# haasn/libplacebo

Measured on AMD Instinct MI355X. Metric: Mpixels/s (and frames/s) for EWA-Lánczos 1080p→4K + HDR tonemap, 1/2/4/8 GPU, higher is better.
Workload: dtype f32; 1 GPU; ewa_1080p_to_4k_hdr_tonemap; src=1920x1080 rgba16, dst=3840x2160 rgba16, pool=10, api=pl_render_image, measured=output Mpixels/s through pl_render_image, one independent stream per GPU, render_errors=0, parallelism=1 independent stream(s), one per GPU

## Files before the change

### libplacebo_amd/csrc/hip/backend.h

```cpp
#ifndef PLH_BACKEND_H_
#define PLH_BACKEND_H_

#include <stddef.h>
#include <stdint.h>

#include "plh_device.h"

#ifdef __cplusplus
extern "C" {
#endif

struct plh_dev_info {
    char name[256];
    char arch[64];
    int compute_units;
    int wavefront_size;
    size_t lds_per_block;
    size_t total_mem;
    int clock_khz;
    uint8_t uuid[16];
    int pci_domain, pci_bus, pci_device;
};

int plh_dev_count(void);
const char *plh_strerror(int err);
int plh_dev_open(int device, struct plh_dev_info *info);
int plh_stream_create(int device, plh_stream *out);
int plh_stream_device(plh_stream s, int *cus);
int plh_kernel_needs_lds(const void *kernel, plh_stream s, size_t bytes, uint64_t *done);
const void *plh_pqseg_tables(plh_stream s, const float consts[5]);
void plh_stream_destroy(plh_stream s);
int plh_stream_sync(plh_stream s);
int plh_stream_idle(plh_stream s);

void *plh_malloc(int device, size_t size);
void plh_free(void *ptr);
void *plh_host_alloc(size_t size);
void *plh_host_alloc_coherent(size_t size);
void plh_host_free(void *ptr);

int plh_copy2d_h2d(plh_stream s, void *dst, size_t dpitch, const void *src, size_t spitch,
                   size_t row_bytes, size_t rows);
int plh_copy2d_d2h(plh_stream s, void *dst, size_t dpitch, const void *src, size_t spitch,
                   size_t row_bytes, size_t rows);
int plh_copy2d_d2d(plh_stream s, void *dst, size_t dpitch, const void *src, size_t spitch,
// ... 27 lines not shown
```

### libplacebo_amd/csrc/hip/backend.hip

```cpp
#include <hip/hip_runtime.h>
#include <string.h>

#include "backend.h"
#include "devmath.hiph"

#define CHK(x) do { hipError_t e_ = (x); if (e_ != hipSuccess) return -(int) e_; } while (0)

extern "C" {

int plh_dev_count(void)
{
    int n = 0;
    if (hipGetDeviceCount(&n) != hipSuccess)
        return 0;
    return n;
}

const char *plh_strerror(int err)
{
    if (err == -1000)
        return "LDS tile does not fit";
    if (err == -1003)
        return "frame mixing ops need a plain (nearest / bilinear) sampler";
    if (err == -1005)
// ... 296 lines not shown

extern "C" int plh_launch_clear_tiles(plh_stream s, const struct plh_view *dst, const float c0[4],
                                      const float c1[4], float kx, float ky)
{
    const dim3 block(64, 4), grid((dst->w + 63) / 64, (dst->h + 3) / 4);
    const float4_t a = { c0[0], c0[1], c0[2], c0[3] }, b = { c1[0], c1[1], c1[2], c1[3] };
    hipLaunchKernelGGL(k_clear_tiles, grid, block, 0, (hipStream_t) s, *dst, a, b, kx, ky);
    const hipError_t err = hipGetLastError();
    return err == hipSuccess ? 0 : -(int) err;
}

#include <math.h>
#include <mutex>
#include "pqseg.hiph"

static double pqseg_oetf(double x, double m1, double c3, double m2)
{
    const double a = (double) PQ_A;
    const double y = x > 0.0 ? pow(x, m1) : 0.0;
    const double w = a * (1.0 - y) / (1.0 + c3 * y);
    return exp(m2 * log1p(-w));
}

static double pqseg_eotf(double v, double c3, double inv_m2, double inv_m1)
{
    const double a = (double) PQ_A;
    if (!(v > 0.0))
        return 0.0;
    const double u = -expm1(log(v) * inv_m2);
    double inner = (a - u) / (a + c3 * u);
    if (!(inner > 0.0))
        return 0.0;
    return pow(inner, inv_m1);
}

static void pqseg_fit(const double node[4], const double f[4], float out[4])
{
    double d[4] = { f[0], f[1], f[2], f[3] };
    for (int j = 1; j < 4; j++) {
        for (int i = 3; i >= j; i--)
            d[i] = (d[i] - d[i - 1]) / (node[i] - node[i - j]);
    }
    double c[4] = { d[3], 0.0, 0.0, 0.0 };
    int deg = 0;
    for (int j = 2; j >= 0; j--) {
// ... 1 lines not shown
        for (int i = 0; i <= deg; i++) {
            n[i] += c[i];
            n[i + 1] -= c[i] * node[j];
        }
        deg++;
        n[deg] += d[j];
        for (int i = 0; i <= deg; i++)
            c[i] = n[i];
    }
    out[0] = (float) c[3];
    out[1] = (float) c[2];
    out[2] = (float) c[1];
    out[3] = (float) c[0];
}

static void plh_pqseg_build(const float consts[5], float *out)
{
    const double m1 = consts[0], c3 = consts[1], m2 = consts[2], inv_m2 = consts[3], inv_m1 = consts[4];
    double cheb[4];
    for (int k = 0; k < 4; k++)
        cheb[k] = 0.5 - 0.5 * cos((2 * k + 1) * M_PI / 8.0);
    for (int s = 0; s < PQSEG_O_N; s++) {
        double f[4];
        for (int k = 0; k < 4; k++)
            f[k] = pqseg_oetf(exp2((double) (PQSEG_O_T0 + s) + cheb[k]), m1, c3, m2);
        pqseg_fit(cheb, f, out + 4 * s);
    }
    float *eo = out + 4 * PQSEG_O_N;
    for (int s = 0; s < PQSEG_E_N; s++) {
        const bool lo = s < PQSEG_E_LO_N;
        const double h = lo ? (double) PQSEG_E_SPLIT / (128.0 * PQSEG_E_LO_N) : 1.0 / 128.0;
        const double v0 = lo ? s * h : (s - PQSEG_E_LO_N + PQSEG_E_SPLIT) * h;
        const double first[4] = { 0.0, 0.3, 0.65, 0.95 };
        const double *node = s == 0 ? first : cheb;
        double f[4];
        for (int k = 0; k < 4; k++)
            f[k] = pqseg_eotf(v0 + h * node[k], c3, inv_m2, inv_m1);
        pqseg_fit(node, f, eo + 4 * s);
    }
}

extern "C" __attribute__((visibility("default")))
void plh_test_pqseg_build(const float consts[5], float *out)
{
    plh_pqseg_build(consts, out);
}

struct pqseg_slot { int dev; float consts[5]; void *ptr; };
static std::mutex g_pqseg_mutex;
static pqseg_slot g_pqseg[16];
static int g_pqseg_n;

extern "C" const void *plh_pqseg_tables(plh_stream s, const float consts[5])
{
    const int dev = plh_stream_device(s, NULL);
    std::lock_guard<std::mutex> lock(g_pqseg_mutex);
    for (int i = 0; i < g_pqseg_n; i++) {
        if (g_pqseg[i].dev == dev && !memcmp(g_pqseg[i].consts, consts, sizeof(g_pqseg[i].consts)))
            return g_pqseg[i].ptr;
    }
    if (g_pqseg_n == 16)
        return NULL;
    static float host[PQSEG_N * 4];
    plh_pqseg_build(consts, host);
    int cur = dev;
    (void) hipGetDevice(&cur);
    if (cur != dev && hipSetDevice(dev) != hipSuccess)
        return NULL;
    void *p = NULL;
    bool ok = hipMalloc(&p, PQSEG_BYTES) == hipSuccess;
    ok = ok && hipMemcpy(p, host, PQSEG_BYTES, hipMemcpyHostToDevice) == hipSuccess;
    if (cur != dev)
        (void) hipSetDevice(cur);
    if (!ok) {
        if (p)
            (void) hipFree(p);
        p = NULL;
    }
    pqseg_slot &e = g_pqseg[g_pqseg_n++];
    e.dev = dev;
    memcpy(e.consts, consts, sizeof(e.consts));
    e.ptr = p;
    return p;
}

__global__ __launch_bounds__(256)
void k_test_pqseg(const float *in, float *out, int n, int which, const void *tables, pq_consts k)
{
    extern __shared__ __attribute__((aligned(16))) unsigned char pqt_smem[];
    pq_seg_stage(pqt_smem, tables, 0, threadIdx.x, 256);
    __syncthreads();
    const pq_seg seg = pq_seg_view(pqt_smem, 0, threadIdx.x & 63u, true);
    const int i = blockIdx.x * 256 + threadIdx.x;
    float v[1] = { in[min(i, n - 1)] };
    if (which == 0)
        pq_eotf_seg<1>(v, seg, k);
// ... 29 lines not shown
```

### libplacebo_amd/csrc/hip/k_peak.hip

```cpp
#include "colorops.hiph"
#include "samplers.hiph"

#define PEAK_BW 16
#define PEAK_BH 16
#define PEAK_SLICES 12
#define PEAK_HIST_BINS 64
#define PQ_BITS 14
#define HIST_BITS 7
#define HIST_BIAS (1 << (HIST_BITS - 1))

struct peak_buf {
    uint32_t frame_wg_count[PEAK_SLICES];
    uint32_t frame_wg_active[PEAK_SLICES];
    uint32_t frame_sum_pq[PEAK_SLICES];
    uint32_t frame_max_pq[PEAK_SLICES];
    uint32_t frame_hist[PEAK_SLICES][PEAK_HIST_BINS];
};

DEV uint32_t wave_sum(uint32_t v)
{
    for (int off = 32; off > 0; off >>= 1)
        v += __shfl_xor(v, off, 64);
    return v;
}
// ... 31 lines not shown
#define PEAK_WAVES 4
#define PL_MIN_INT(a, b) ((a) < (b) ? (a) : (b))
#define PEAK_NPX 4

struct peak_pq_consts {
    float inv_m2, c1, c2, c3, inv_m1, gain, out_scale, out_add;
    int flags;
};

DEV peak_pq_consts peak_load_pq(const plh_op &op)
{
    const float *f = op.f;
    return { f[2], f[3], f[4], f[5], f[6], f[7], f[0], f[1], op.i1 };
}

DEV void peak_linearize_pq(float4_t &c, const peak_pq_consts &k)
{
    float v[3] = { c.x, c.y, c.z };
#pragma unroll
    for (int i = 0; i < 3; i++) {
        if (k.flags & PLH_TRC_CLAMP0)
            v[i] = fmaxf(v[i], 0.0f);
        const float p = plh_powf(v[i], k.inv_m2);
        const float r = div1(fmaxf(p - k.c1, 0.0f), __builtin_fmaf(-k.c3, p, k.c2));
        v[i] = plh_powf(r, k.inv_m1) * k.gain;
        if (k.flags & PLH_TRC_RESCALE)
            v[i] = k.out_scale * v[i] + k.out_add;
    }
    c.x = v[0]; c.y = v[1]; c.z = v[2];
}

DEV void peak_linearize(float4_t &c, const plh_op &op)
{
    if (op.i0 != TRC_PQ) {
        op_linearize(c, op);
        return;
    }
    peak_linearize_pq(c, peak_load_pq(op));
}

struct peak_consts {
    float luma[3], white, m1, c1, c2, c3, m2, cutoff;
};

DEV peak_consts peak_load_consts(const plh_op &op)
{
    const float *e = (const float *) op.ptr2;
    return { { e[0], e[1], e[2] }, e[3], e[4], e[5], e[6], e[7], e[8], e[9] };
}

DEV uint32_t peak_luma_pq14(const float4_t &c, const peak_consts &e)
{
    float luma = e.luma[0] * c.x + e.luma[1] * c.y + e.luma[2] * c.z;
    luma *= e.white;
    luma = plh_powf(plh_clamp(luma, 0.0f, 1.0f), e.m1);
    luma = div1(e.c1 + e.c2 * luma, 1.0f + e.c3 * luma);
    luma = plh_powf(luma, e.m2);
    const float cutoff = e.cutoff;
    if (cutoff != 0.0f) {
        const float t = plh_clamp(div1(luma, cutoff), 0.0f, 1.0f);
        luma *= t * t * (3.0f - 2.0f * t);
    }
    return (uint32_t) (16383.0f * luma);
}

DEV uint32_t peak_pq14(const float4_t &c_in, const plh_op &op, const peak_consts &e)
{
    float4_t c = c_in;
    if (op.i0 != TRC_LINEAR)
        peak_linearize(c, op);
    return peak_luma_pq14(c, e);
}

DEV uint32_t peak_pq14(const float4_t &c_in, const plh_op &op)
{
    return peak_pq14(c_in, op, peak_load_consts(op));
}

DEV void wave_lds_fence()
{
    __builtin_amdgcn_fence(__ATOMIC_ACQ_REL, "wavefront");
    __builtin_amdgcn_wave_barrier();
}

DEV void peak_measure(const float4_t (&c)[PEAK_NPX], const plh_op &op, uint32_t *hist,
                      uint32_t wg_idx, void *scratch)
{
    const int lane = threadIdx.x & 63;
    const float cutoff = ((const float *) op.ptr2)[9];
    uint32_t y_pq[PEAK_NPX];
#pragma unroll
    for (int k = 0; k < PEAK_NPX; k++)
        y_pq[k] = peak_pq14(c[k], op);

    if (op.i2) {
        hist[lane] = 0u;
        wave_lds_fence();
#pragma unroll
        for (int k = 0; k < PEAK_NPX; k++) {
            int bin = (int) y_pq[k] >> (PQ_BITS - HIST_BITS);
            bin -= HIST_BIAS;
            bin = min(max(bin, 0), PEAK_HIST_BINS - 1);
            const int first = __shfl(bin, 0, 64);
            if (__all(bin == first)) {
                if (lane == 0)
                    atomicAdd(&hist[bin], 64u);
            } else {
                atomicAdd(&hist[bin], 1u);
// ... 100 lines not shown
    } else if (s.type != PLH_SAMPLE_NONE) {
#pragma unroll
        for (int k = 0; k < PEAK_NPX; k++)
            c[k] = run_sampler_pk(s, px[k], py[k]);
    }

    int pk_op = p.num_ops;
    for (int i = 0; i < p.num_ops; i++) {
        if (p.ops[i].kind == PLH_OP_PEAK_DETECT) {
            pk_op = i;
            break;
        }
    }
    apply_ops_n<PEAK_NPX, false, LITE>(c, p.ops, 0, pk_op, fcs);
    if (pk_op < p.num_ops) {
        peak_measure(c, p.ops[pk_op], hists[wave], wg_idx, p.peak_scratch);
        apply_ops_n<PEAK_NPX, false, LITE>(c, p.ops, pk_op + 1, p.num_ops, fcs);
    }

    if (!p.dst.ptr)
        return;
    int sx[PEAK_NPX], sy[PEAK_NPX];
    bool ok[PEAK_NPX];
#pragma unroll
    for (int k = 0; k < PEAK_NPX; k++) {
        sx[k] = p.base_x + p.dir_x * (p.transpose ? idy[k] : idx[k]);
        sy[k] = p.base_y + p.dir_y * (p.transpose ? idx[k] : idy[k]);
        ok[k] = p.out_scale[0] * (float) idx[k] < 1.0f && p.out_scale[1] * (float) idy[k] < 1.0f &&
                sx[k] >= 0 && sy[k] >= 0 && sx[k] < p.dst.w && sy[k] < p.dst.h;
    }
    plh_store_n<PEAK_NPX>(p.dst, sx, sy, ok, c, p.nt_store);
// ... 78 lines not shown
                continue;
            uint32_t o[4];
#pragma unroll
            for (int i = 0; i < 2; i++) {
                const float4_t &t = c[2 * k + i];
                o[2 * i] = (uint32_t) plh_f2h(t.x) | ((uint32_t) plh_f2h(t.y) << 16);
                o[2 * i + 1] = (uint32_t) plh_f2h(t.z) | ((uint32_t) plh_f2h(t.w) << 16);
            }
            char *d = (char *) p.dst.ptr + (size_t) y * p.dst.pitch + (size_t) x0 * 8;
            if (x0 + 1 < w)
                *(uint4 *) d = make_uint4(o[0], o[1], o[2], o[3]);
            else
                *(uint2 *) d = make_uint2(o[0], o[1]);
        }
    }
    peak_measure(c, o_pk, hists[wave], wg_idx, p.peak_scratch);
}

#define PEAK_PAD 32
#define PEAK_TICKETS 4096
DEV uint32_t *peak_pad_word(uint32_t *scratch, uint32_t i)
{
    return i < 4 * PEAK_SLICES ? scratch + i * PEAK_PAD : scratch + 4 * PEAK_SLICES * PEAK_PAD + (i - 4 * PEAK_SLICES);
}

template <bool F16SRC, int STORE, bool PQ>
__global__ __launch_bounds__(64 * PEAK_WAVES)
void k_peak_tiles(const plh_pass p_)
{
    const plh_pass &p = plh_kernarg_pass();
    const plh_sampler_args &s = p.s;
    __shared__ uint32_t blk[4 + PEAK_HIST_BINS];
    const int lane = threadIdx.x & 63;
    const int wave = __builtin_amdgcn_readfirstlane(threadIdx.x >> 6);
    int w = p.width, h = p.height;
    const int tiles_x = (w + PEAK_BW - 1) / PEAK_BW;
    const int tiles_y = (h + PEAK_BH - 1) / PEAK_BH;
    const uint32_t ntiles = (uint32_t) (tiles_x * tiles_y);
    const uint32_t slice = blockIdx.x % PEAK_SLICES, bs = blockIdx.x / PEAK_SLICES;
    const uint32_t stride = (gridDim.x / PEAK_SLICES) * PEAK_WAVES;
    const uint32_t per_slice = (ntiles + PEAK_SLICES - 1 - slice) / PEAK_SLICES;
    const bool has_map = STORE != 2 && p.num_ops == 2;
    const plh_op &o_map = p.ops[0], &o_pk = p.ops[STORE == 2 ? 0 : p.num_ops - 1];
    plh_op feat, flin;
    bool feat_lin = false;
    if constexpr (STORE == 2) {
        const plh_op &of = p.ops[p.num_ops - 1], &ol = p.ops[1];
// ... 2 lines not shown
        for (int k = 0; k < 14; k++)
            feat.f[k] = of.f[k];
        flin.i1 = ol.i1;
#pragma unroll
        for (int k = 0; k < 8; k++)
            flin.f[k] = ol.f[k];
        asm volatile("" : "+s"(feat.f[0]), "+s"(feat.f[1]), "+s"(feat.f[2]), "+s"(feat.f[3]), "+s"(feat.f[4]),
                          "+s"(feat.f[5]), "+s"(feat.f[6]), "+s"(feat.f[7]), "+s"(feat.f[8]), "+s"(feat.f[9]),
                          "+s"(feat.f[10]), "+s"(feat.f[11]), "+s"(feat.f[12]), "+s"(feat.f[13]));
        asm volatile("" : "+s"(flin.i1), "+s"(flin.f[0]), "+s"(flin.f[1]), "+s"(flin.f[2]), "+s"(flin.f[3]),
                          "+s"(flin.f[4]), "+s"(flin.f[5]), "+s"(flin.f[6]), "+s"(flin.f[7]));
    }
    auto uni = [](float v) { return __int_as_float(__builtin_amdgcn_readfirstlane(__float_as_int(v))); };
    const peak_consts pcv = peak_load_consts(o_pk);
    peak_consts pc = { { uni(pcv.luma[0]), uni(pcv.luma[1]), uni(pcv.luma[2]) }, uni(pcv.white), uni(pcv.m1),
                       uni(pcv.c1), uni(pcv.c2), uni(pcv.c3), uni(pcv.m2), uni(pcv.cutoff) };
    peak_pq_consts pq = peak_load_pq(o_pk);
    int use_hist = o_pk.i2;
    const float rtx = 1.0f / (float) tiles_x;
    uintptr_t sp = (uintptr_t) s.src.ptr, dp = (uintptr_t) p.dst.ptr;
    int spitch = s.src.pitch, dpitch = p.dst.pitch;
    int map_n = 4;
    float nt1 = 0.0f, nt2 = 0.0f, nt3 = 1.0f;
    if (has_map) {
        map_n = o_map.i1;
        nt1 = o_map.f[1]; nt2 = o_map.f[2]; nt3 = o_map.f[3];
    }
    asm volatile("" : "+s"(w), "+s"(h), "+s"(use_hist), "+s"(sp), "+s"(dp), "+s"(spitch),
                      "+s"(dpitch), "+s"(map_n), "+s"(nt1), "+s"(nt2), "+s"(nt3));
    asm volatile("" : "+s"(pc.luma[0]), "+s"(pc.luma[1]), "+s"(pc.luma[2]), "+s"(pc.white), "+s"(pc.m1),
                      "+s"(pc.c1), "+s"(pc.c2), "+s"(pc.c3), "+s"(pc.m2), "+s"(pc.cutoff));
    asm volatile("" : "+s"(pq.inv_m2), "+s"(pq.c1), "+s"(pq.c2), "+s"(pq.c3), "+s"(pq.inv_m1), "+s"(pq.gain),
                      "+s"(pq.out_scale), "+s"(pq.out_add), "+s"(pq.flags));
    typedef __attribute__((address_space(1))) const plh_u32x4 g_u32x4;
    typedef __attribute__((address_space(1))) plh_u32x4 g_u32x4_w;
    typedef __attribute__((address_space(1))) plh_u32x2 g_u32x2_w;

    if (threadIdx.x < 4 + PEAK_HIST_BINS)
        blk[threadIdx.x] = 0u;
    __syncthreads();

    auto origin = [&](uint32_t j, int &x0, int &y0) {
        const uint32_t t = PEAK_SLICES * j + slice;
        const int ty = (int) (((float) t + 0.5f) * rtx);
        const int tx = (int) t - ty * tiles_x;
        x0 = tx * PEAK_BW + 2 * (lane & 7);
        y0 = ty * PEAK_BH + (lane >> 3);
    };
    uint32_t n_wg = 0, n_lit = 0, sum_pq = 0, lane_max = 0, black = 0;
    for (uint32_t j = bs * PEAK_WAVES + (uint32_t) wave; j < per_slice; j += stride) {
        int x0, y0;
        origin(j, x0, y0);
        const int px = min(x0, w - 2);
        uint32_t lane_sum = 0, nblack = 0;
        auto fetch = [&](int k) {
            return *(g_u32x4 *) (sp + (size_t) min(y0 + 8 * k, h - 1) * (size_t) spitch + (size_t) px * 8);
        };
        auto row = [&](int k, plh_u32x4 v) {
            const int y = y0 + 8 * k;
            if (x0 + 1 >= w) {
                v.x = v.z; v.y = v.w;
            }
            const uint32_t q[4] = { v.x, v.y, v.z, v.w };
            float4_t c[2];
#pragma unroll
            for (int i = 0; i < 2; i++) {
                const uint32_t lo = q[2 * i], hi = q[2 * i + 1];
                float4_t t;
                if (F16SRC)
                    t = { plh_h2f(lo & 0xffff), plh_h2f(lo >> 16), plh_h2f(hi & 0xffff), plh_h2f(hi >> 16) };
                else
                    t = { plh_un16(lo & 0xffff), plh_un16(lo >> 16), plh_un16(hi & 0xffff), plh_un16(hi >> 16) };
                if (map_n < 4) t.w = nt3;
                if (map_n < 3) t.z = nt2;
                if (map_n < 2) t.y = nt1;
                c[i] = t;
            }
            if constexpr (STORE == 2) {
                float4_t t[2] = { c[0], c[1] };
                if (feat_lin) {
                    float v6[6] = { t[0].x, t[0].y, t[0].z, t[1].x, t[1].y, t[1].z };
                    lin_values<TRC_PQ>(v6, flin);
                    t[0].x = v6[0]; t[0].y = v6[1]; t[0].z = v6[2];
                    t[1].x = v6[3]; t[1].y = v6[4]; t[1].z = v6[5];
                }
                uint32_t o[2];
#pragma unroll
                for (int i = 0; i < 2; i++) {
                    op_features(t[i], feat);
                    o[i] = plh_f2h(t[i].x);
// ... 5 lines not shown
                    *(__attribute__((address_space(1))) uint16_t *) d = (uint16_t) o[0];
            }
            if constexpr (STORE == 1) {
                uint32_t o[4];
#pragma unroll
                for (int i = 0; i < 2; i++) {
                    o[2 * i] = (uint32_t) plh_f2h(c[i].x) | ((uint32_t) plh_f2h(c[i].y) << 16);
                    o[2 * i + 1] = (uint32_t) plh_f2h(c[i].z) | ((uint32_t) plh_f2h(c[i].w) << 16);
                }
                const uintptr_t d = dp + (size_t) y * (size_t) dpitch + (size_t) x0 * 8;
                if (y < h && x0 + 1 < w)
                    *(g_u32x4_w *) d = (plh_u32x4) { o[0], o[1], o[2], o[3] };
                else if (y < h && x0 < w)
                    *(g_u32x2_w *) d = (plh_u32x2) { o[0], o[1] };
            }
#pragma unroll
            for (int i = 0; i < 2; i++) {
                if (PQ)
                    peak_linearize_pq(c[i], pq);
                const uint32_t y_pq = peak_luma_pq14(c[i], pc);
                if (use_hist) {
                    int bin = (int) y_pq >> (PQ_BITS - HIST_BITS);
                    bin -= HIST_BIAS;
                    bin = min(max(bin, 0), PEAK_HIST_BINS - 1);
                    const int first = __builtin_amdgcn_readfirstlane(bin);
                    if (__all(bin == first)) {
                        if (lane == 0)
                            atomicAdd(&blk[4 + bin], 64u);
                    } else {
                        atomicAdd(&blk[4 + bin], 1u);
                    }
                }
                lane_sum += y_pq;
                lane_max = max(lane_max, y_pq);
                if (pc.cutoff != 0.0f)
                    nblack += (uint32_t) __popcll(__ballot(y_pq == 0u));
            }
        };
        if constexpr (STORE == 2) {
            const plh_u32x4 v0 = fetch(0), v1 = fetch(1);
            row(0, v0);
            row(1, v1);
        } else {
#pragma unroll 1
            for (int k = 0; k < 2; k++)
                row(k, fetch(k));
        }
        const uint32_t wg_sum = wave_sum_dpp(lane_sum);
        const uint32_t num = PEAK_BW * PEAK_BH - nblack;
        n_wg += 1u;
        n_lit += min(num, 1u);
        if (nblack == 0u)
            sum_pq += wg_sum / (PEAK_BW * PEAK_BH);
        else if (num > 0u)
            sum_pq += wg_sum / num;
        black += nblack;
    }

    const uint32_t wmax = wave_max_dpp(lane_max);
    if (lane == 0 && n_wg) {
        atomicAdd(&blk[0], n_wg);
// ... 116 lines not shown
    if (!last)
        return;
    __threadfence();
    for (uint32_t i = threadIdx.x; i < PLH_PEAK_WORDS; i += blockDim.x) {
        const uint32_t v = __hip_atomic_load(&dst[i], __ATOMIC_RELAXED, __HIP_MEMORY_SCOPE_AGENT);
        __hip_atomic_store(&mailbox[i], v, __ATOMIC_RELAXED, __HIP_MEMORY_SCOPE_SYSTEM);
    }
    __threadfence_system();
    __syncthreads();
    if (threadIdx.x == 0) {
        *counter = 0u;
        __hip_atomic_store(&mailbox[PLH_PEAK_WORDS], ticket, __ATOMIC_RELEASE, __HIP_MEMORY_SCOPE_SYSTEM);
    }
}

int plh_launch_peak(hipStream_t stream, const plh_pass *pass)
{
    const int tiles = ((pass->width + PEAK_BW - 1) / PEAK_BW) * ((pass->height + PEAK_BH - 1) / PEAK_BH);
    const dim3 block(64 * PEAK_WAVES);
    const dim3 grid((tiles + PEAK_WAVES - 1) / PEAK_WAVES);
    if (!pass->peak_buf || !pass->peak_scratch)
        return -1002;
    int pk_op = pass->num_ops;
    for (int i = 0; i < pass->num_ops; i++) {
        if (pass->ops[i].kind == PLH_OP_PEAK_DETECT) {
            pk_op = i;
            break;
        }
    }
    const int trc = pk_op < pass->num_ops ? pass->ops[pk_op].i0 : -1;
    const bool feat_target = pass->dst.ptr && pass->dst.fmt == PLH_FMT_R16F;
    const bool feat_ok = !feat_target || pass->num_ops == 2 || pass->ops[1].i0 == TRC_PQ;
    if (peak_fast_applies(pass) && plh_switch(PLH_SW_PEAK_TILES) && feat_ok && pass->width >= 2 &&
        (trc == TRC_PQ || trc == TRC_LINEAR)) {
        const bool f16 = pass->s.src.fmt == PLH_FMT_RGBA16F, store = pass->dst.ptr != NULL, pq = trc == TRC_PQ;
        const int per_slice = (tiles + PEAK_SLICES - 1) / PEAK_SLICES;
        int groups = (per_slice + 2 * PEAK_WAVES - 1) / (2 * PEAK_WAVES);
        groups = groups < 1 ? 1 : groups > 170 ? 170 : groups;
        const dim3 tgrid(PEAK_SLICES * groups);
#define PEAK_TILES_GO(F, S, Q) PLH_LAUNCH_LAST((k_peak_tiles<F, S, Q>), tgrid, block, 0, stream, *pass)
        if (f16 && feat_target) { if (pq) PEAK_TILES_GO(true, 2, true); else PEAK_TILES_GO(true, 2, false); }
        else if (feat_target)   { if (pq) PEAK_TILES_GO(false, 2, true); else PEAK_TILES_GO(false, 2, false); }
        else if (f16 && store)  { if (pq) PEAK_TILES_GO(true, 1, true); else PEAK_TILES_GO(true, 1, false); }
        else if (f16)           { if (pq) PEAK_TILES_GO(true, 0, true); else PEAK_TILES_GO(true, 0, false); }
        else if (store)         { if (pq) PEAK_TILES_GO(false, 1, true); else PEAK_TILES_GO(false, 1, false); }
        else                    { if (pq) PEAK_TILES_GO(false, 0, true); else PEAK_TILES_GO(false, 0, false); }
// ... 26 lines not shown
```

### libplacebo_amd/csrc/hip/plh_device.h

```cpp
#ifndef PLH_DEVICE_H_
#define PLH_DEVICE_H_

#include <stdint.h>

#include "plh_switch.h"

#ifdef __cplusplus
extern "C" {
#endif

enum plh_fmt {
    PLH_FMT_NONE = 0,
    PLH_FMT_R8, PLH_FMT_RG8, PLH_FMT_RGBA8,
    PLH_FMT_R16, PLH_FMT_RG16, PLH_FMT_RGBA16,
    PLH_FMT_R16F, PLH_FMT_RG16F, PLH_FMT_RGBA16F,
    PLH_FMT_R32F, PLH_FMT_RG32F, PLH_FMT_RGBA32F,
    PLH_FMT_COUNT
};

struct plh_view {
    void *ptr;
    int32_t w, h;
    int32_t pitch;
    int32_t fmt;
// ... 235 lines not shown
    int32_t dir_x, dir_y;
    int32_t width, height;
    float out_scale[2];
    int32_t transpose;
    int32_t frag_x0, frag_y0;
    int32_t cell_padx, cell_pady;
    int32_t nt_store;

    struct plh_fast_epi epi;
    struct plh_map_chain chain;

    void *peak_buf;
    void *peak_scratch;
    void *peak_mailbox;
    uint32_t peak_ticket;

    struct plh_deint_args deint;
    struct plh_distort_args distort;
};

static inline int plh_pass_covers_source(const struct plh_pass *pass)
{
    const struct plh_sampler_args *s = &pass->s;
    return pass->width == s->src.w && pass->height == s->src.h &&
        s->pos[0][0] == 0.0f && s->pos[0][1] == 0.0f && s->pos[3][0] == 1.0f && s->pos[3][1] == 1.0f &&
        s->pos[1][0] == 1.0f && s->pos[1][1] == 0.0f && s->pos[2][0] == 0.0f && s->pos[2][1] == 1.0f;
}

static inline int plh_pass_plain_target(const struct plh_pass *pass)
{
// ... 91 lines not shown
```

### libplacebo_amd/csrc/hip/plh_switch.h

```cpp
#ifndef PLH_SWITCH_H_
#define PLH_SWITCH_H_

#ifdef __cplusplus
extern "C" {
#endif

#define PLH_SWITCHES(X) \
    X(ASYNC_MEASURE,   "PL_HIP_ASYNC_MEASURE",   -1, "0 | 1 override pl_hip_params.async_measure (the measuring pass on a second stream); unset: the parameter") \
    X(NO_FUSION,       "PL_HIP_NO_FUSION",       -1, "1: the renderer records the reference's separate passes; 0: fuses wherever it is valid; unset: where it also pays") \
    X(FUSED_FEATURES,  "PL_HIP_FUSED_FEATURES",   1, "0: the contrast-recovery feature map as its own pass instead of a side output of the plane pass") \
    X(NT_STORE,        "PL_HIP_NT_STORE",         1, "0: plain stores to unorm targets instead of streaming (non-temporal) ones") \
    X(POLAR_MFMA,      "PL_HIP_POLAR_MFMA",       1, "0: every polar pass on the bit-exact sequential-fma kernels instead of the matrix-pipe ones") \
    X(POLAR_PER_PIXEL, "PL_HIP_POLAR_PER_PIXEL",  0, "1: polar weights evaluated per pixel (k_polar) instead of from phase-class tables (k_polar_pp)") \
    X(MX_PERSIST,      "PL_HIP_MX_PERSIST",       1, "0: k_polar_mx (a workgroup per tile) instead of k_polar_mxp (persistent workgroups)") \
    X(MAP_CHAIN,       "PL_HIP_MAP_CHAIN",        1, "0: colour-management ops walked by the interpreter instead of the straight-line chain") \
    X(PQ_SEGMENTS,     "PL_HIP_PQ_SEGMENTS",      1, "0: the chain's PQ pair in closed form instead of piecewise cubics in LDS") \
    X(PQ_SEG_COPIES,   "PL_HIP_PQ_SEG_COPIES",    1, "1 | 2 | 4 | 8 | 16 copies of every piece of those cubics in k_polar_mx's LDS") \
    X(CHAIN_SHAPE,     "PL_HIP_CHAIN_SHAPE",      1, "0: k_polar_mx's generic chain instance always, instead of its shape-specialised one for HDR10 -> SDR passes (bit-identical)") \
    X(PASS_NATIVE,     "PL_HIP_PASS_NATIVE",      1, "0: 1:1 passes on k_pass_generic instead of k_pass_native / k_pass_chain / k_pass_merge / k_pass_mix") \
    X(BILIN_ITERS,     "PL_HIP_BILIN_ITERS",      1, "1 | 2 | 4 cells per lane of k_bilinear_fast; 0: k_pass_generic instead of it and of k_nearest_fast") \
    X(BILIN_TABLES,    "PL_HIP_BILIN_TABLES",     0, "1: the 2x bilinear upscale on k_bilinear_tab (per-axis tables) instead of k_bilinear_fast") \
    X(BILIN_STRIP,     "PL_HIP_BILIN_STRIP",      0, "1: the 2x bilinear upscale on k_bilinear_strip (a 16-byte load per cell) instead of k_bilinear_fast") \
    X(ORTHO_FAST,      "PL_HIP_ORTHO_FAST",       1, "0: separable passes on k_ortho instead of k_ortho_fast") \
    X(LOWPASS_FUSED,   "PL_HIP_LOWPASS_FUSED",    1, "0: the feature map's low-pass as two ortho passes instead of the one k_lowpass2 launch") \
    X(DEBAND_FAST,     "PL_HIP_DEBAND_FAST",      1, "0: debanding on k_deband instead of k_deband_fast / k_deband_lds") \
    X(DEBAND_LDS,      "PL_HIP_DEBAND_LDS",       1, "0: k_deband_fast (fetches from memory) instead of k_deband_lds (window staged in LDS)") \
    X(PEAK_FAST,       "PL_HIP_PEAK_FAST",        1, "0: peak detection on k_pass_peak (the op interpreter) instead of k_peak_tiles / k_peak_fast") \
    X(PEAK_TILES,      "PL_HIP_PEAK_TILES",       1, "0: k_peak_fast + k_peak_fold (two launches) instead of k_peak_tiles (folded on chip)") \
    X(PASS_TRACE,      "PL_HIP_PASS_TRACE",       0, "1: one line per pass launch on stderr: sampler, formats, op list (tools/time_ops.py)") \
    X(PP_ROWS,         "PL_HIP_PP_ROWS",          0, "profiling aid: output rows per lane of k_polar_pp; 0: chosen from the geometry") \
    X(PP_DEBUG,        "PL_HIP_PP_DEBUG",         0, "profiling aid, bit mask: 1 no taps, 2 no verification, 4 no stores, 8 no tile loads")

enum plh_switch_id {
#define PLH_SWITCH_ID(id, name, def, doc) PLH_SW_##id,
    PLH_SWITCHES(PLH_SWITCH_ID)
#undef PLH_SWITCH_ID
    PLH_SW_COUNT
};

int plh_switch(enum plh_switch_id id);

#ifdef __cplusplus
}
#endif
// ... 3 lines not shown
```

### libplacebo_amd/csrc/host/shader_color.c

```c
#include <math.h>
#include <stdlib.h>
#include <string.h>
#include <time.h>

#include <libplacebo/shaders/colorspace.h>

#include "shaders_priv.h"
#include "cache_priv.h"
#include "colorspace_priv.h"

#define MIXF(a, b, x) ((x) * (b) + (1 - (x)) * (a))

const struct pl_sigmoid_params pl_sigmoid_default_params = { PL_SIGMOID_DEFAULTS };
const struct pl_peak_detect_params pl_peak_detect_default_params = { PL_PEAK_DETECT_DEFAULTS };
const struct pl_peak_detect_params pl_peak_detect_high_quality_params = { PL_PEAK_DETECT_HQ_DEFAULTS };
const struct pl_color_map_params pl_color_map_default_params = { PL_COLOR_MAP_DEFAULTS };
const struct pl_color_map_params pl_color_map_high_quality_params = { PL_COLOR_MAP_HQ_DEFAULTS };

static struct plh_op *simple_op(pl_shader sh, int kind, const char *listing)
{
    struct plh_op *op = sh_op(sh, kind);
    if (op)
        sh_listf(sh, "%s\n", listing);
    return op;
// ... 845 lines not shown
        const size_t size = (size_t) PLH_PEAK_COPIES * sizeof(struct peak_buf_data) + 64;
        void *zeros = calloc(1, size);
        obj->peak.scratch = zeros ? pl_buf_create(gpu, pl_buf_params(
            .size = size, .storable = true, .initial_data = zeros)) : NULL;
        free(zeros);
        if (!obj->peak.scratch)
            return false;
        obj->peak.tables_seq = plh_gpu_stamp(gpu, 0);
    }
    sh->aux_after = obj->peak.tables_seq;
    sh->pass.peak_buf = pl_hip_buf_ptr(obj->peak.buf);
    sh->pass.peak_scratch = pl_hip_buf_ptr(obj->peak.scratch);
    obj->peak.ticket = obj->peak.ticket + 1 ? obj->peak.ticket + 1 : 1;
    sh->pass.peak_mailbox = obj->peak.mirror;
    sh->pass.peak_ticket = obj->peak.ticket;
    sh->detect_peak = true;
    sh->peak_state = *state;
    sh_hold(sh, *state);

    sh_describef(sh, "peak detection");
    sh_listf(sh, "detect_peak(trc=%s, histogram=%d, cutoff=%g)\n",
             pl_color_transfer_name(csp.transfer), (int) use_histogram, consts[9]);
    return true;
}

bool pl_get_detected_hdr_metadata(const pl_shader_obj state, struct pl_hdr_metadata *out)
{
    if (!state || state->type != PL_SHADER_OBJ_COLOR_MAP)
        return false;

// ... 300 lines not shown
```

Baseline: 90830 Mpixels/s.

## Use piecewise-cubic PQ tables for peak detection instead of closed-form pow

Peak detection now replaces the PQ EOTF linearisation and the PQ OETF luma encoding with lookups into precomputed piecewise-cubic tables, staged into LDS inside k_peak_tiles. Values outside the table range fall back to the closed-form pow path, selected per wave with a ballot. The table builder gains per-curve a1/a2 parameters so the tables match the pass's constants. The change also adds a waves-per-eu hint, moves some values to scalar registers, and multiplies by a reciprocal cutoff in place of a divide. It costs LDS per block, adds table staging, and gives slightly different numerics from the closed form.

Measured after the change: 91550 Mpixels/s (median of 6 runs). About the same (+0.8%).

```diff
diff --git a/libplacebo_amd/csrc/hip/backend.h b/libplacebo_amd/csrc/hip/backend.h
--- a/libplacebo_amd/csrc/hip/backend.h
+++ b/libplacebo_amd/csrc/hip/backend.h
@@ -29,6 +29,7 @@
 int plh_stream_device(plh_stream s, int *cus);
 int plh_kernel_needs_lds(const void *kernel, plh_stream s, size_t bytes, uint64_t *done);
 const void *plh_pqseg_tables(plh_stream s, const float consts[5]);
+const void *plh_pqseg_tables_a(plh_stream s, const float consts[5], const double a[4]);
 void plh_stream_destroy(plh_stream s);
 int plh_stream_sync(plh_stream s);
 int plh_stream_idle(plh_stream s);
diff --git a/libplacebo_amd/csrc/hip/backend.hip b/libplacebo_amd/csrc/hip/backend.hip
--- a/libplacebo_amd/csrc/hip/backend.hip
+++ b/libplacebo_amd/csrc/hip/backend.hip
@@ -334,21 +334,19 @@
 #include <mutex>
 #include "pqseg.hiph"
 
-static double pqseg_oetf(double x, double m1, double c3, double m2)
-{
-    const double a = (double) PQ_A;
+static double pqseg_oetf(double x, double m1, double c3, double m2, double a1, double a2)
+{
     const double y = x > 0.0 ? pow(x, m1) : 0.0;
-    const double w = a * (1.0 - y) / (1.0 + c3 * y);
+    const double w = a1 == a2 ? a1 * (1.0 - y) / (1.0 + c3 * y) : (a1 - a2 * y) / (1.0 + c3 * y);
     return exp(m2 * log1p(-w));
 }
 
-static double pqseg_eotf(double v, double c3, double inv_m2, double inv_m1)
-{
-    const double a = (double) PQ_A;
+static double pqseg_eotf(double v, double c3, double inv_m2, double inv_m1, double a1, double a2)
+{
     if (!(v > 0.0))
         return 0.0;
     const double u = -expm1(log(v) * inv_m2);
-    double inner = (a - u) / (a + c3 * u);
+    double inner = (a1 - u) / (a2 + c3 * u);
     if (!(inner > 0.0))
         return 0.0;
     return pow(inner, inv_m1);
@@ -380,7 +378,7 @@
     out[3] = (float) c[0];
 }
 
-static void plh_pqseg_build(const float consts[5], float *out)
+static void plh_pqseg_build(const float consts[5], const double a[4], float *out)
 {
     const double m1 = consts[0], c3 = consts[1], m2 = consts[2], inv_m2 = consts[3], inv_m1 = consts[4];
     double cheb[4];
@@ -389,7 +387,7 @@
     for (int s = 0; s < PQSEG_O_N; s++) {
         double f[4];
         for (int k = 0; k < 4; k++)
-            f[k] = pqseg_oetf(exp2((double) (PQSEG_O_T0 + s) + cheb[k]), m1, c3, m2);
+            f[k] = pqseg_oetf(exp2((double) (PQSEG_O_T0 + s) + cheb[k]), m1, c3, m2, a[0], a[1]);
         pqseg_fit(cheb, f, out + 4 * s);
     }
     float *eo = out + 4 * PQSEG_O_N;
@@ -401,7 +399,7 @@
         const double *node = s == 0 ? first : cheb;
         double f[4];
         for (int k = 0; k < 4; k++)
-            f[k] = pqseg_eotf(v0 + h * node[k], c3, inv_m2, inv_m1);
+            f[k] = pqseg_eotf(v0 + h * node[k], c3, inv_m2, inv_m1, a[2], a[3]);
         pqseg_fit(node, f, eo + 4 * s);
     }
 }
@@ -409,26 +407,41 @@
 extern "C" __attribute__((visibility("default")))
 void plh_test_pqseg_build(const float consts[5], float *out)
 {
-    plh_pqseg_build(consts, out);
-}
-
-struct pqseg_slot { int dev; float consts[5]; void *ptr; };
+    const double a[4] = { (double) PQ_A, (double) PQ_A, (double) PQ_A, (double) PQ_A };
+    plh_pqseg_build(consts, a, out);
+}
+
+extern "C" __attribute__((visibility("default")))
+void plh_test_pqseg_build_a(const float consts[5], const double a[4], float *out)
+{
+    plh_pqseg_build(consts, a, out);
+}
+
+struct pqseg_slot { int dev; float consts[5]; double a[4]; void *ptr; };
 static std::mutex g_pqseg_mutex;
 static pqseg_slot g_pqseg[16];
 static int g_pqseg_n;
 
 extern "C" const void *plh_pqseg_tables(plh_stream s, const float consts[5])
 {
+    return plh_pqseg_tables_a(s, consts, NULL);
+}
+
+extern "C" const void *plh_pqseg_tables_a(plh_stream s, const float consts[5], const double a_[4])
+{
+    const double pq_a[4] = { (double) PQ_A, (double) PQ_A, (double) PQ_A, (double) PQ_A };
+    const double *a = a_ ? a_ : pq_a;
     const int dev = plh_stream_device(s, NULL);
     std::lock_guard<std::mutex> lock(g_pqseg_mutex);
     for (int i = 0; i < g_pqseg_n; i++) {
-        if (g_pqseg[i].dev == dev && !memcmp(g_pqseg[i].consts, consts, sizeof(g_pqseg[i].consts)))
+        if (g_pqseg[i].dev == dev && !memcmp(g_pqseg[i].consts, consts, sizeof(g_pqseg[i].consts)) &&
+            !memcmp(g_pqseg[i].a, a, sizeof(g_pqseg[i].a)))
             return g_pqseg[i].ptr;
     }
     if (g_pqseg_n == 16)
         return NULL;
     static float host[PQSEG_N * 4];
-    plh_pqseg_build(consts, host);
+    plh_pqseg_build(consts, a, host);
     int cur = dev;
     (void) hipGetDevice(&cur);
     if (cur != dev && hipSetDevice(dev) != hipSuccess)
@@ -446,6 +459,7 @@
     pqseg_slot &e = g_pqseg[g_pqseg_n++];
     e.dev = dev;
     memcpy(e.consts, consts, sizeof(e.consts));
+    memcpy(e.a, a, sizeof(e.a));
     e.ptr = p;
     return p;
 }
diff --git a/libplacebo_amd/csrc/hip/k_peak.hip b/libplacebo_amd/csrc/hip/k_peak.hip
--- a/libplacebo_amd/csrc/hip/k_peak.hip
+++ b/libplacebo_amd/csrc/hip/k_peak.hip
@@ -1,5 +1,8 @@
 #include "colorops.hiph"
 #include "samplers.hiph"
+#include "pqseg.hiph"
+#include "backend.h"
+#include <string.h>
 
 #define PEAK_BW 16
 #define PEAK_BH 16
@@ -69,6 +72,13 @@
     return { f[2], f[3], f[4], f[5], f[6], f[7], f[0], f[1], op.i1 };
 }
 
+DEV float peak_eotf_pow(float v, const peak_pq_consts &k)
+{
+    const float p = plh_powf(v, k.inv_m2);
+    const float r = div1(fmaxf(p - k.c1, 0.0f), __builtin_fmaf(-k.c3, p, k.c2));
+    return plh_powf(r, k.inv_m1);
+}
+
 DEV void peak_linearize_pq(float4_t &c, const peak_pq_consts &k)
 {
     float v[3] = { c.x, c.y, c.z };
@@ -76,60 +86,130 @@
     for (int i = 0; i < 3; i++) {
         if (k.flags & PLH_TRC_CLAMP0)
             v[i] = fmaxf(v[i], 0.0f);
-        const float p = plh_powf(v[i], k.inv_m2);
-        const float r = div1(fmaxf(p - k.c1, 0.0f), __builtin_fmaf(-k.c3, p, k.c2));
-        v[i] = plh_powf(r, k.inv_m1) * k.gain;
+        v[i] = peak_eotf_pow(v[i], k) * k.gain;
         if (k.flags & PLH_TRC_RESCALE)
             v[i] = k.out_scale * v[i] + k.out_add;
     }
     c.x = v[0]; c.y = v[1]; c.z = v[2];
 }
 
-DEV void peak_linearize(float4_t &c, const plh_op &op)
+struct peak_seg {
+    const unsigned char *base;
+    bool on;
+    float vmax;
+};
+#define PEAK_SEG_VMAX (PQSEG_E_VMAX - 1.0f / 8388608.0f)
+#define PEAK_SEG_O      ((uint32_t) -PQSEG_O_T0 * 16u)
+#define PEAK_SEG_E      ((uint32_t) PQSEG_O_N * 16u)
+#define PEAK_SEG_E_HI   ((uint32_t) (PQSEG_O_N + PQSEG_E_LO_N - PQSEG_E_SPLIT) * 16u)
+
+template <bool GLOBAL>
+DEV float4 peak_eotf_piece(float vc, const unsigned char *base, float &u)
+{
+    const float p = vc * 128.0f;
+    const bool fine = p < (float) PQSEG_E_SPLIT;
+    const float pos = fine ? p * (float) (PQSEG_E_LO_N / PQSEG_E_SPLIT) : p;
+    u = __builtin_amdgcn_fractf(pos);
+    return pq_seg_piece<GLOBAL>(base + PEAK_SEG_E + ((((uint32_t) pos) << 4) + (fine ? 0u : PEAK_SEG_E_HI - PEAK_SEG_E)));
+}
+
+template <bool GLOBAL>
+DEV float4 peak_oetf_piece(float x, const unsigned char *base, float &u)
+{
+    const float pos = fmaxf(__builtin_amdgcn_logf(x), (float) PQSEG_O_T0);
+    u = __builtin_amdgcn_fractf(pos);
+    return pq_seg_piece<GLOBAL>(base + (int) (PEAK_SEG_O + (uint32_t) ((int) __builtin_floorf(pos) << 4)));
+}
+
+template <bool GLOBAL>
+DEV void peak_linearize_pq(float4_t &c, const peak_pq_consts &k, const peak_seg &t)
+{
+    if (!t.on) {
+        peak_linearize_pq(c, k);
+        return;
+    }
+    float v[3] = { c.x, c.y, c.z }, u[3], r[3];
+    float4 cf[3];
+    uint64_t in[3];
+#pragma unroll
+    for (int i = 0; i < 3; i++) {
+        if (k.flags & PLH_TRC_CLAMP0)
+            v[i] = fmaxf(v[i], 0.0f);
+        const float vc = __builtin_amdgcn_fmed3f(v[i], 0.0f, t.vmax);
+        in[i] = __builtin_amdgcn_ballot_w64(vc == v[i]);
+        cf[i] = peak_eotf_piece<GLOBAL>(vc, t.base, u[i]);
+        __builtin_amdgcn_sched_barrier(0);
+    }
+#pragma unroll
+    for (int i = 0; i < 3; i++)
+        r[i] = pq_seg_cubic(cf[i], u[i]);
+    if (__builtin_expect(!__builtin_amdgcn_inverse_ballot_w64(in[0] & in[1] & in[2]), false)) {
+#pragma unroll
+        for (int i = 0; i < 3; i++) {
+            const float pw = peak_eotf_pow(v[i], k);
+            r[i] = __builtin_amdgcn_inverse_ballot_w64(in[i]) ? r[i] : pw;
+        }
+    }
+#pragma unroll
+    for (int i = 0; i < 3; i++) {
+        v[i] = r[i] * k.gain;
+        if (k.flags & PLH_TRC_RESCALE)
+            v[i] = k.out_scale * v[i] + k.out_add;
+    }
+    c.x = v[0]; c.y = v[1]; c.z = v[2];
+}
+
+template <bool GLOBAL>
+DEV void peak_linearize(float4_t &c, const plh_op &op, const peak_seg &t)
 {
     if (op.i0 != TRC_PQ) {
         op_linearize(c, op);
         return;
     }
-    peak_linearize_pq(c, peak_load_pq(op));
+    peak_linearize_pq<GLOBAL>(c, peak_load_pq(op), t);
 }
 
 struct peak_consts {
     float luma[3], white, m1, c1, c2, c3, m2, cutoff;
+    float rcutoff;
 };
 
 DEV peak_consts peak_load_consts(const plh_op &op)
 {
     const float *e = (const float *) op.ptr2;
-    return { { e[0], e[1], e[2] }, e[3], e[4], e[5], e[6], e[7], e[8], e[9] };
-}
-
-DEV uint32_t peak_luma_pq14(const float4_t &c, const peak_consts &e)
+    return { { e[0], e[1], e[2] }, e[3], e[4], e[5], e[6], e[7], e[8], e[9], __builtin_amdgcn_rcpf(e[9]) };
+}
+
+template <bool GLOBAL>
+DEV uint32_t peak_luma_pq14(const float4_t &c, const peak_consts &e, const peak_seg &t)
 {
     float luma = e.luma[0] * c.x + e.luma[1] * c.y + e.luma[2] * c.z;
     luma *= e.white;
-    luma = plh_powf(plh_clamp(luma, 0.0f, 1.0f), e.m1);
-    luma = div1(e.c1 + e.c2 * luma, 1.0f + e.c3 * luma);
-    luma = plh_powf(luma, e.m2);
+    luma = plh_clamp(luma, 0.0f, 1.0f);
+    if (t.on) {
+        float u;
+        const float4 cf = peak_oetf_piece<GLOBAL>(luma, t.base, u);
+        luma = pq_seg_cubic(cf, u);
+    } else {
+        luma = plh_powf(luma, e.m1);
+        luma = div1(e.c1 + e.c2 * luma, 1.0f + e.c3 * luma);
+        luma = plh_powf(luma, e.m2);
+    }
     const float cutoff = e.cutoff;
     if (cutoff != 0.0f) {
-        const float t = plh_clamp(div1(luma, cutoff), 0.0f, 1.0f);
-        luma *= t * t * (3.0f - 2.0f * t);
+        const float q = luma * e.rcutoff;
+        const float s = plh_clamp(__builtin_fmaf(__builtin_fmaf(-q, cutoff, luma), e.rcutoff, q), 0.0f, 1.0f);
+        luma *= s * s * (3.0f - 2.0f * s);
     }
     return (uint32_t) (16383.0f * luma);
 }
 
-DEV uint32_t peak_pq14(const float4_t &c_in, const plh_op &op, const peak_consts &e)
+DEV uint32_t peak_pq14(const float4_t &c_in, const plh_op &op, const peak_consts &e, const peak_seg &t)
 {
     float4_t c = c_in;
     if (op.i0 != TRC_LINEAR)
-        peak_linearize(c, op);
-    return peak_luma_pq14(c, e);
-}
-
-DEV uint32_t peak_pq14(const float4_t &c_in, const plh_op &op)
-{
-    return peak_pq14(c_in, op, peak_load_consts(op));
+        peak_linearize<true>(c, op, t);
+    return peak_luma_pq14<true>(c, e, t);
 }
 
 DEV void wave_lds_fence()
@@ -139,14 +219,16 @@
 }
 
 DEV void peak_measure(const float4_t (&c)[PEAK_NPX], const plh_op &op, uint32_t *hist,
-                      uint32_t wg_idx, void *scratch)
+                      uint32_t wg_idx, void *scratch, const void *segp)
 {
     const int lane = threadIdx.x & 63;
-    const float cutoff = ((const float *) op.ptr2)[9];
+    const peak_consts e = peak_load_consts(op);
+    const float cutoff = e.cutoff;
+    const peak_seg seg = { (const unsigned char *) segp, segp != nullptr, PEAK_SEG_VMAX };
     uint32_t y_pq[PEAK_NPX];
 #pragma unroll
     for (int k = 0; k < PEAK_NPX; k++)
-        y_pq[k] = peak_pq14(c[k], op);
+        y_pq[k] = peak_pq14(c[k], op, e, seg);
 
     if (op.i2) {
         hist[lane] = 0u;
@@ -277,7 +359,7 @@
     }
     apply_ops_n<PEAK_NPX, false, LITE>(c, p.ops, 0, pk_op, fcs);
     if (pk_op < p.num_ops) {
-        peak_measure(c, p.ops[pk_op], hists[wave], wg_idx, p.peak_scratch);
+        peak_measure(c, p.ops[pk_op], hists[wave], wg_idx, p.peak_scratch, p.peak_seg);
         apply_ops_n<PEAK_NPX, false, LITE>(c, p.ops, pk_op + 1, p.num_ops, fcs);
     }
 
@@ -386,8 +468,10 @@
                 *(uint2 *) d = make_uint2(o[0], o[1]);
         }
     }
-    peak_measure(c, o_pk, hists[wave], wg_idx, p.peak_scratch);
-}
+    peak_measure(c, o_pk, hists[wave], wg_idx, p.peak_scratch, p.peak_seg);
+}
+
+template <bool B> struct peak_tag { static constexpr bool value = B; };
 
 #define PEAK_PAD 32
 #define PEAK_TICKETS 4096
@@ -397,12 +481,13 @@
 }
 
 template <bool F16SRC, int STORE, bool PQ>
-__global__ __launch_bounds__(64 * PEAK_WAVES)
+__global__ __launch_bounds__(64 * PEAK_WAVES) __attribute__((amdgpu_waves_per_eu(STORE == 2 ? 8 : 1, 8)))
 void k_peak_tiles(const plh_pass p_)
 {
     const plh_pass &p = plh_kernarg_pass();
     const plh_sampler_args &s = p.s;
     __shared__ uint32_t blk[4 + PEAK_HIST_BINS];
+    __shared__ __attribute__((aligned(16))) unsigned char segl[PQSEG_BYTES];
     const int lane = threadIdx.x & 63;
     const int wave = __builtin_amdgcn_readfirstlane(threadIdx.x >> 6);
     int w = p.width, h = p.height;
@@ -435,10 +520,10 @@
     auto uni = [](float v) { return __int_as_float(__builtin_amdgcn_readfirstlane(__float_as_int(v))); };
     const peak_consts pcv = peak_load_consts(o_pk);
     peak_consts pc = { { uni(pcv.luma[0]), uni(pcv.luma[1]), uni(pcv.luma[2]) }, uni(pcv.white), uni(pcv.m1),
-                       uni(pcv.c1), uni(pcv.c2), uni(pcv.c3), uni(pcv.m2), uni(pcv.cutoff) };
+                       uni(pcv.c1), uni(pcv.c2), uni(pcv.c3), uni(pcv.m2), uni(pcv.cutoff), uni(pcv.rcutoff) };
     peak_pq_consts pq = peak_load_pq(o_pk);
     int use_hist = o_pk.i2;
-    const float rtx = 1.0f / (float) tiles_x;
+    const float rtx = uni(1.0f / (float) tiles_x);
     uintptr_t sp = (uintptr_t) s.src.ptr, dp = (uintptr_t) p.dst.ptr;
     int spitch = s.src.pitch, dpitch = p.dst.pitch;
     int map_n = 4;
@@ -450,23 +535,34 @@
     asm volatile("" : "+s"(w), "+s"(h), "+s"(use_hist), "+s"(sp), "+s"(dp), "+s"(spitch),
                       "+s"(dpitch), "+s"(map_n), "+s"(nt1), "+s"(nt2), "+s"(nt3));
     asm volatile("" : "+s"(pc.luma[0]), "+s"(pc.luma[1]), "+s"(pc.luma[2]), "+s"(pc.white), "+s"(pc.m1),
-                      "+s"(pc.c1), "+s"(pc.c2), "+s"(pc.c3), "+s"(pc.m2), "+s"(pc.cutoff));
-    asm volatile("" : "+s"(pq.inv_m2), "+s"(pq.c1), "+s"(pq.c2), "+s"(pq.c3), "+s"(pq.inv_m1), "+s"(pq.gain),
-                      "+s"(pq.out_scale), "+s"(pq.out_add), "+s"(pq.flags));
+                      "+s"(pc.c1), "+s"(pc.c2), "+s"(pc.c3), "+s"(pc.m2), "+s"(pc.cutoff), "+s"(pc.rcutoff));
+    if constexpr (STORE != 2)
+        asm volatile("" : "+s"(pq.inv_m2), "+s"(pq.c1), "+s"(pq.c2), "+s"(pq.c3), "+s"(pq.inv_m1),
+                          "+s"(pq.out_scale), "+s"(pq.out_add));
+    asm volatile("" : "+s"(pq.gain), "+s"(pq.flags));
     typedef __attribute__((address_space(1))) const plh_u32x4 g_u32x4;
     typedef __attribute__((address_space(1))) plh_u32x4 g_u32x4_w;
     typedef __attribute__((address_space(1))) plh_u32x2 g_u32x2_w;
 
     if (threadIdx.x < 4 + PEAK_HIST_BINS)
         blk[threadIdx.x] = 0u;
+    const bool seg_on = p.peak_seg != nullptr;
+    if (seg_on)
+        pq_seg_stage(segl, p.peak_seg, 0, threadIdx.x, 64 * PEAK_WAVES);
+    float seg_vmax = PEAK_SEG_VMAX;
+    asm volatile("" : "+s"(seg_vmax));
+    const peak_seg seg = { segl, seg_on, seg_vmax };
+    const bool shape = seg_on && (!PQ || pq.flags == PLH_TRC_CLAMP0) && map_n >= 3;
     __syncthreads();
 
     auto origin = [&](uint32_t j, int &x0, int &y0) {
         const uint32_t t = PEAK_SLICES * j + slice;
-        const int ty = (int) (((float) t + 0.5f) * rtx);
+        const int ty = __builtin_amdgcn_readfirstlane((int) (((float) t + 0.5f) * rtx));
         const int tx = (int) t - ty * tiles_x;
-        x0 = tx * PEAK_BW + 2 * (lane & 7);
-        y0 = ty * PEAK_BH + (lane >> 3);
+        int l = lane;
+        asm volatile("" : "+v"(l));
+        x0 = tx * PEAK_BW + 2 * (l & 7);
+        y0 = ty * PEAK_BH + (l >> 3);
     };
     uint32_t n_wg = 0, n_lit = 0, sum_pq = 0, lane_max = 0, black = 0;
     for (uint32_t j = bs * PEAK_WAVES + (uint32_t) wave; j < per_slice; j += stride) {
@@ -477,7 +573,8 @@
         auto fetch = [&](int k) {
             return *(g_u32x4 *) (sp + (size_t) min(y0 + 8 * k, h - 1) * (size_t) spitch + (size_t) px * 8);
         };
-        auto row = [&](int k, plh_u32x4 v) {
+        auto row = [&](int k, plh_u32x4 v, auto shape_tag) {
+            constexpr bool SHAPE = decltype(shape_tag)::value;
             const int y = y0 + 8 * k;
             if (x0 + 1 >= w) {
                 v.x = v.z; v.y = v.w;
@@ -493,8 +590,10 @@
                 else
                     t = { plh_un16(lo & 0xffff), plh_un16(lo >> 16), plh_un16(hi & 0xffff), plh_un16(hi >> 16) };
                 if (map_n < 4) t.w = nt3;
-                if (map_n < 3) t.z = nt2;
-                if (map_n < 2) t.y = nt1;
+                if constexpr (!SHAPE) {
+                    if (map_n < 3) t.z = nt2;
+                    if (map_n < 2) t.y = nt1;
+                }
                 c[i] = t;
             }
             if constexpr (STORE == 2) {
@@ -530,11 +629,19 @@
                 else if (y < h && x0 < w)
                     *(g_u32x2_w *) d = (plh_u32x2) { o[0], o[1] };
             }
+            __builtin_amdgcn_sched_barrier(0);
+            peak_pq_consts pqk = pq;
+            peak_seg segk = seg;
+            segk.on = SHAPE;
+            if constexpr (SHAPE)
+                pqk.flags = PLH_TRC_CLAMP0;
 #pragma unroll
             for (int i = 0; i < 2; i++) {
                 if (PQ)
-                    peak_linearize_pq(c[i], pq);
-                const uint32_t y_pq = peak_luma_pq14(c[i], pc);
+                    peak_linearize_pq<false>(c[i], pqk, segk);
+                const uint32_t y_pq = peak_luma_pq14<false>(c[i], pc, segk);
+                if (i == 0)
+                    asm volatile("" : "+v"(c[1].x), "+v"(c[1].y), "+v"(c[1].z) : "v"(y_pq));
                 if (use_hist) {
                     int bin = (int) y_pq >> (PQ_BITS - HIST_BITS);
                     bin -= HIST_BIAS;
@@ -553,14 +660,18 @@
                     nblack += (uint32_t) __popcll(__ballot(y_pq == 0u));
             }
         };
-        if constexpr (STORE == 2) {
+        if (shape) {
+#pragma unroll 1
+            for (int k = 0; k < 2; k++)
+                row(k, fetch(k), peak_tag<true>());
+        } else if constexpr (STORE == 2) {
             const plh_u32x4 v0 = fetch(0), v1 = fetch(1);
-            row(0, v0);
-            row(1, v1);
+            row(0, v0, peak_tag<false>());
+            row(1, v1, peak_tag<false>());
         } else {
 #pragma unroll 1
             for (int k = 0; k < 2; k++)
-                row(k, fetch(k));
+                row(k, fetch(k), peak_tag<false>());
         }
         const uint32_t wg_sum = wave_sum_dpp(lane_sum);
         const uint32_t num = PEAK_BW * PEAK_BH - nblack;
@@ -707,8 +818,43 @@
     }
 }
 
-int plh_launch_peak(hipStream_t stream, const plh_pass *pass)
-{
+static bool plh_peak_seg_consts(const plh_op *op, const float pq[5], float k5[5], double a[4])
+{
+    const double M1 = 2610.0 / 16384, M2 = 2523.0 / 32, C1 = 3424.0 / 4096, C2 = 2413.0 / 128, C3 = 2392.0 / 128;
+    auto st2084 = [](double v, double ref) { return fabs(v - ref) <= 4e-6 * ref; };
+    if (!(st2084(pq[0], M1) && st2084(pq[1], C1) && st2084(pq[2], C2) && st2084(pq[3], C3) && st2084(pq[4], M2)))
+        return false;
+    float inv_m2 = 1.0f / pq[4], inv_m1 = 1.0f / pq[0];
+    a[0] = a[2] = 1.0 - (double) pq[1];
+    a[1] = a[3] = (double) pq[2] - (double) pq[3];
+    if (op->i0 == TRC_PQ) {
+        const float *f = op->f;
+        if (!(st2084(f[2], 1.0 / M2) && st2084(f[3], C1) && st2084(f[4], C2) && f[5] == pq[3] && st2084(f[6], 1.0 / M1)))
+            return false;
+        inv_m2 = f[2];
+        inv_m1 = f[6];
+        a[2] = 1.0 - (double) f[3];
+        a[3] = (double) f[4] - (double) f[5];
+    }
+    k5[0] = pq[0]; k5[1] = pq[3]; k5[2] = pq[4]; k5[3] = inv_m2; k5[4] = inv_m1;
+    return true;
+}
+
+extern "C" __attribute__((visibility("default")))
+int plh_test_peak_seg_consts(int trc, const float *f, const float *pq, float *k5, double *a)
+{
+    plh_op op = {};
+    op.kind = PLH_OP_PEAK_DETECT;
+    op.i0 = trc;
+    for (int i = 0; i < PLH_OP_NF; i++)
+        op.f[i] = f[i];
+    return plh_peak_seg_consts(&op, pq, k5, a);
+}
+
+int plh_launch_peak(hipStream_t stream, const plh_pass *pass_)
+{
+    plh_pass local = *pass_;
+    const plh_pass *pass = &local;
     const int tiles = ((pass->width + PEAK_BW - 1) / PEAK_BW) * ((pass->height + PEAK_BH - 1) / PEAK_BH);
     const dim3 block(64 * PEAK_WAVES);
     const dim3 grid((tiles + PEAK_WAVES - 1) / PEAK_WAVES);
@@ -723,6 +869,16 @@
     }
     const int trc = pk_op < pass->num_ops ? pass->ops[pk_op].i0 : -1;
     const bool feat_target = pass->dst.ptr && pass->dst.fmt == PLH_FMT_R16F;
+    float k5[5];
+    double k_a[4];
+    local.peak_seg = NULL;
+    if (pk_op < pass->num_ops && plh_switch(PLH_SW_PEAK_SEG) &&
+        (trc != TRC_PQ || pass->ops[pk_op].i1 == PLH_TRC_CLAMP0) &&
+        !(pk_op > 0 && pass->ops[0].kind == PLH_OP_PLANE_MAP && pass->ops[0].i1 < 3) &&
+        plh_peak_seg_consts(&pass->ops[pk_op], pass->peak_pq, k5, k_a))
+        local.peak_seg = plh_pqseg_tables_a((plh_stream) stream, k5, k_a);
+    if (plh_switch(PLH_SW_PASS_TRACE))
+        fprintf(stderr, "[plh] peak: %s\n", local.peak_seg ? "PQ pieces" : "closed form");
     const bool feat_ok = !feat_target || pass->num_ops == 2 || pass->ops[1].i0 == TRC_PQ;
     if (peak_fast_applies(pass) && plh_switch(PLH_SW_PEAK_TILES) && feat_ok && pass->width >= 2 &&
         (trc == TRC_PQ || trc == TRC_LINEAR)) {
diff --git a/libplacebo_amd/csrc/hip/plh_device.h b/libplacebo_amd/csrc/hip/plh_device.h
--- a/libplacebo_amd/csrc/hip/plh_device.h
+++ b/libplacebo_amd/csrc/hip/plh_device.h
@@ -273,6 +273,8 @@
     void *peak_scratch;
     void *peak_mailbox;
     uint32_t peak_ticket;
+    float peak_pq[5];
+    const void *peak_seg;
 
     struct plh_deint_args deint;
     struct plh_distort_args distort;
diff --git a/libplacebo_amd/csrc/hip/plh_switch.h b/libplacebo_amd/csrc/hip/plh_switch.h
--- a/libplacebo_amd/csrc/hip/plh_switch.h
+++ b/libplacebo_amd/csrc/hip/plh_switch.h
@@ -27,7 +27,8 @@
     X(DEBAND_LDS,      "PL_HIP_DEBAND_LDS",       1, "0: k_deband_fast (fetches from memory) instead of k_deband_lds (window staged in LDS)") \
     X(PEAK_FAST,       "PL_HIP_PEAK_FAST",        1, "0: peak detection on k_pass_peak (the op interpreter) instead of k_peak_tiles / k_peak_fast") \
     X(PEAK_TILES,      "PL_HIP_PEAK_TILES",       1, "0: k_peak_fast + k_peak_fold (two launches) instead of k_peak_tiles (folded on chip)") \
-    X(PASS_TRACE,      "PL_HIP_PASS_TRACE",       0, "1: one line per pass launch on stderr: sampler, formats, op list (tools/time_ops.py)") \
+    X(PEAK_SEG,        "PL_HIP_PEAK_SEG",         1, "0: the measuring pass's PQ pair in closed form (native pow) instead of the piecewise cubics, value by value") \
+    X(PASS_TRACE,     "PL_HIP_PASS_TRACE",       0, "1: one line per pass launch on stderr: sampler, formats, op list (tools/time_ops.py)") \
     X(PP_ROWS,         "PL_HIP_PP_ROWS",          0, "profiling aid: output rows per lane of k_polar_pp; 0: chosen from the geometry") \
     X(PP_DEBUG,        "PL_HIP_PP_DEBUG",         0, "profiling aid, bit mask: 1 no taps, 2 no verification, 4 no stores, 8 no tile loads")
 
diff --git a/libplacebo_amd/csrc/host/shader_color.c b/libplacebo_amd/csrc/host/shader_color.c
--- a/libplacebo_amd/csrc/host/shader_color.c
+++ b/libplacebo_amd/csrc/host/shader_color.c
@@ -883,6 +883,8 @@
     obj->peak.ticket = obj->peak.ticket + 1 ? obj->peak.ticket + 1 : 1;
     sh->pass.peak_mailbox = obj->peak.mirror;
     sh->pass.peak_ticket = obj->peak.ticket;
+    memcpy(sh->pass.peak_pq, &consts[4], sizeof(sh->pass.peak_pq));
+    sh->pass.peak_seg = NULL;
     sh->detect_peak = true;
     sh->peak_state = *state;
     sh_hold(sh, *state);
```
